# avishkarsaha/learning-adaptive-neighborhoods-for-gnns

Measured on AMD Instinct MI355X. Metric: DGG adj-build+SpMM fwd/bwd edges/sec & achieved HBM GB/s, N=100k d=128 k=32, higher is better.
Workload: dtype f32; 1 GPU; synthetic all-pairs DGG N=100000 d=128 h=64 k~32.3 K=64, u-v-dist/x/k_times_edge_prob, Gumbel(0,0.3) perturbation, + normalize + GCNConv(128,64), fwd+bwd; nodes=100000, feat=128, latent=64, parallelism=row-shard x1, rows_per_rank=100000, hipgraph=True, noise=ranked

## Files before the change

### learning-adaptive-neighborhoods-for-gnns_amd/csrc/dgg_scatter.hip

```cpp
#include "dgg_common.h"
#include "dgg_api_internal.h"
#include "../../include/dgg_hip_next.h"

using namespace dgg;

namespace {

constexpr int BS = 128;
constexpr int PR = 256;

struct PartHdr {
    int *bstart, *cursor;
    int2 *tmp;
    int *slot;
    int2 *recs;
    int *cstart;
};
__host__ __device__ inline size_t align256(size_t x) { return (x + 255) / 256 * 256; }
inline PartHdr part_layout(void *ws, int64_t nb, int64_t nrec) {
    char *w = reinterpret_cast<char *>(ws);
    PartHdr p;
    p.bstart = reinterpret_cast<int *>(w);
    p.cursor = reinterpret_cast<int *>(w + align256((size_t)(nb + 1) * 4));
    p.tmp = reinterpret_cast<int2 *>(w + align256((size_t)(nb + 1) * 4) + align256((size_t)nb * 4));
// ... 70 lines not shown

__global__ __launch_bounds__(1024) void part_sort(const int *__restrict__ bstart, const int2 *__restrict__ tmp, int K,
                                                 int2 *__restrict__ recs, int *__restrict__ slotmap) {
    __shared__ int cnt[BS], base[BS];
    const int tid = threadIdx.x, b = blockIdx.x;
    const int e0 = bstart[b], e1 = bstart[b + 1];
    if (tid < BS) cnt[tid] = 0;
    __syncthreads();
    for (int e = e0 + tid; e < e1; e += 1024) atomicAdd(&cnt[tmp[e].y - b * BS], 1);
    __syncthreads();
    if (tid < 64) {
        const int c0 = cnt[2 * tid], c1 = cnt[2 * tid + 1];
        int incl = c0 + c1;
#pragma unroll
        for (int off = 1; off < 64; off <<= 1) {
            const int v = __shfl_up(incl, off, 64);
            if (tid >= off) incl += v;
        }
        base[2 * tid] = incl - c0 - c1;
        base[2 * tid + 1] = incl - c1;
    }
    __syncthreads();
    if (tid < BS) cnt[tid] = 0;
    __syncthreads();
    for (int e = e0 + tid; e < e1; e += 1024) {
        const int2 rec = tmp[e];
        const int jl = rec.y - b * BS;
        const int pos = e0 + base[jl] + atomicAdd(&cnt[jl], 1);
        recs[pos] = rec;
        slotmap[(int64_t)(rec.x >> 6) * K + (rec.x & 63)] = pos;
    }
}

__global__ void part_chunk_starts(const int *__restrict__ bstart, int nb, const int2 *__restrict__ recs, int nchunks, int chunk,
                                  int *__restrict__ cstart) {
    const int c = blockIdx.x * blockDim.x + threadIdx.x;
    if (c > nchunks) return;
    const int nnz = bstart[nb];
    const int64_t x = (int64_t)c * chunk;
    int e = x < nnz ? (int)x : nnz;
    if (e > 0) {
        const int lim = e + 48 < nnz ? e + 48 : nnz;
        while (e < lim && recs[e].y == recs[e - 1].y) e++;
        if (e < nnz && recs[e].y == recs[e - 1].y) e = (int)x;
    }
    cstart[c] = e;
}

__global__ __launch_bounds__(1024) void part_scan(int *__restrict__ bstart, int *__restrict__ cursor, int nb) {
    __shared__ int part[1024];
    const int tid = threadIdx.x;
    const int per = (nb + 1023) / 1024;
    const int lo = tid * per, hi = lo + per < nb ? lo + per : nb;
    int s = 0;
    for (int b = lo; b < hi; b++) s += cursor[b];
    part[tid] = s;
    __syncthreads();
    for (int off = 1; off < 1024; off <<= 1) {
        int v = tid >= off ? part[tid - off] : 0;
        __syncthreads();
        part[tid] += v;
        __syncthreads();
    }
    int run = part[tid] - s;
    for (int b = lo; b < hi; b++) {
        const int c = cursor[b];
        bstart[b] = run;
        cursor[b] = run;
        run += c;
    }
    if (tid == 1023) bstart[nb] = part[1023];
}

struct SoftkArgs {
    const float *k, *rs, *dA, *da;
    int mode, normalized;
    float *dval_out, *dk;
    const float *ahat_rows;
    float4 *rowinfo;
    const int *recpos;
    const float *dA_rec;
    const float *ainv;
};
template <int H, int R0, int NB>
__device__ __forceinline__ float edge_rows_group(const float *__restrict__ xp, int64_t gi, int K, int lane, int32_t jl, bool myact,
                                                 bool mine, float gl, float vl, float t, int perturb, const float4 xi, float4 &acc) {
    constexpr int LPR = H / 4, NPI = 64 / LPR, r0 = R0;
    const int c4 = lane % LPR, slot = lane / LPR;
    float4 xj[NB];
#pragma unroll
    for (int b = 0; b < NB; b++) {
        const int r = r0 + b * NPI + slot;
        const int rr = r < 64 ? r : 63;
        const int32_t jb = __shfl(jl, rr, 64);
        const bool ab = __shfl((int)myact, rr, 64) != 0 && r < K;
        xj[b] = *reinterpret_cast<const float4 *>(xp + (ab ? (int64_t)jb : gi) * H + 4 * c4);
    }
    float myd2 = 0.0f;
#pragma unroll
    for (int b = 0; b < NB; b++) {
        const float4 d = make_float4(xi.x - xj[b].x, xi.y - xj[b].y, xi.z - xj[b].z, xi.w - xj[b].w);
        float d2 = d.x * d.x + d.y * d.y + d.z * d.z + d.w * d.w;
        if (LPR > 16) d2 += __uint_as_float(xor_shfl<16>(__float_as_uint(d2), lane));
        if (LPR > 8) d2 += __uint_as_float(xor_shfl<8>(__float_as_uint(d2), lane));
        if (LPR > 4) d2 += __uint_as_float(xor_shfl<4>(__float_as_uint(d2), lane));
        if (LPR > 2) d2 += __uint_as_float(xor_shfl<2>(__float_as_uint(d2), lane));
        d2 += __uint_as_float(xor_shfl<1>(__float_as_uint(d2), lane));
        const float tq = __shfl(d2, (lane % NPI) * LPR, 64);
        if ((lane - r0) / NPI == b && mine) myd2 = tq;
    }
    float mydd = 0.0f;
    if (mine && myact && myd2 != 0.0f) {
        const float dist = sqrtf(myd2);
        const float p = c_exp(t * dist);
        const float dp = perturb ? gl * vl / (p + 1e-8f) : gl;
        mydd = dp * t * p / dist;
    }
#pragma unroll
    for (int b = 0; b < NB; b++) {
        const int r = r0 + b * NPI + slot;
        const float dd = __shfl(mydd, r < 64 ? r : 63, 64);
        const float4 d = make_float4(xi.x - xj[b].x, xi.y - xj[b].y, xi.z - xj[b].z, xi.w - xj[b].w);
        acc.x += dd * d.x; acc.y += dd * d.y; acc.z += dd * d.z; acc.w += dd * d.w;
    }
    return mydd;
}
template <int H, int R0, int NBT, int NB = NBT>
__device__ __forceinline__ float edge_rows_pick(int nbat, const float *__restrict__ xp, int64_t gi, int K, int lane, int32_t jl,
                                                bool myact, bool mine, float gl, float vl, float t, int perturb, const float4 xi, float4 &acc) {
    constexpr int STEP = NBT > 8 ? NBT / 8 : 1;
    if constexpr (NB > STEP) {
        if (nbat <= NB - STEP) return edge_rows_pick<H, R0, NBT, NB - STEP>(nbat, xp, gi, K, lane, jl, myact, mine, gl, vl, t, perturb, xi, acc);
    }
    return edge_rows_group<H, R0, NB>(xp, gi, K, lane, jl, myact, mine, gl, vl, t, perturb, xi, acc);
}

template <int H, bool COEF, int R0>
__device__ __forceinline__ void edge_rows_half(const float *__restrict__ xp, int64_t gi, int K, int lane, int32_t jl, bool myact, float gl, float vl,
                                               float t, int perturb, const float4 xi, float4 &acc, float &mycoef) {
    constexpr int NPI = 64 / (H / 4), NBT = 32 / NPI;
    const bool mine = lane >= R0 && lane < R0 + 32;
    const unsigned long long actmask = __ballot(mine && myact);
    if (actmask == 0ull) return;
    const int nbat = (63 - __clzll(actmask) - R0) / NPI + 1;
    const float mydd = edge_rows_pick<H, R0, NBT>(nbat, xp, gi, K, lane, jl, myact, mine, gl, vl, t, perturb, xi, acc);
    if (COEF && mine) mycoef = mydd;
}

template <int H, bool FUSE, bool PAY = false>
__global__ __launch_bounds__(256) void edge_bwd_rows(const float *__restrict__ xp, int64_t rows, const int32_t *__restrict__ idx,
                                                     const float *__restrict__ val, const float *__restrict__ dval, int K,
                                                     int64_t row0, float t, int perturb, const int *__restrict__ slotmap,
                                                     float *__restrict__ coef, float *__restrict__ dxp, SoftkArgs sk) {
    constexpr int LPR = H / 4;
    constexpr int NPI = 64 / LPR;
    const int lane = threadIdx.x & 63, c4 = lane % LPR, slot = lane / LPR;
    const int64_t i = (int64_t)blockIdx.x * 4 + dgg::wave_id();
    if (i >= rows) return;
    const int64_t gi = row0 + i;
    const int32_t jl = lane < K ? idx[i * K + lane] : -1;
    const float vl = lane < K ? val[i * K + lane] : 0.0f;
    float gl;
    if (FUSE) {
        const int lc = lane < K ? lane : K - 1;
        const bool viamap = PAY && sk.recpos != nullptr;
        float dw = viamap ? 0.0f : sk.dA[i * K + lc];
        const int rpos = viamap ? sk.recpos[i * 64 + lc] : 0;
        const bool live = lane < K && jl >= 0;
        if (sk.normalized) {
            const float rsi = sk.rs[gi];
            const int64_t jx = jl >= 0 ? jl : gi;
            const float ai = __fdiv_rn(1.0f, c_sqrt(rsi));
            const float aj = (PAY && sk.ainv) ? sk.ainv[jx] : __fdiv_rn(1.0f, c_sqrt(sk.rs[jx]));
            float dai = sk.da[gi];
            if (sk.ahat_rows) {
                const float ah = lane < K ? sk.ahat_rows[i * K + lane] : 0.0f;
                if (viamap) dw = sk.dA_rec[ah != 0.0f ? rpos : 0];
                if (PAY && ah == 0.0f) dw = 0.0f;
                float rp = dw * ah;
                rp = wave_sum_dpp(rp, lane);
                dai += rp * sqrtf(rsi);
            }
            const float drs = -0.5f * dai * ai / rsi;
            dw = dw * ai * aj + drs;
            if (PAY && lane == 0) sk.rowinfo[i] = make_float4(ai, drs, sk.k[i], 0.0f);
        } else if (PAY && lane == 0) {
            sk.rowinfo[i] = make_float4(1.0f, 0.0f, sk.k[i], 0.0f);
        }
        const float th = c_tanh((float)lane - sk.k[i]);
        const float f = 1.0f - 0.5f * (1.0f + th);
        const float dfdk = 0.5f * (1.0f - th * th);
        gl = (live && sk.mode == 0) ? dw * f : 0.0f;
        float skp = live ? (sk.mode == 0 ? dw * vl * dfdk : dw * dfdk) : 0.0f;
#pragma unroll
        for (int off = 32; off >= 1; off >>= 1) skp += __shfl_xor(skp, off, 64);
        if (lane == 0) sk.dk[i] = skp;
        if (sk.dval_out && lane < K) sk.dval_out[i * K + lane] = gl;
    } else {
        gl = lane < K ? dval[i * K + lane] : 0.0f;
    }
    const float4 xi = *reinterpret_cast<const float4 *>(xp + gi * H + 4 * c4);
    float4 acc = make_float4(0.0f, 0.0f, 0.0f, 0.0f);
    float mycoef = 0.0f;
    constexpr int NBT = (32 / NPI) < 1 ? 1 : 32 / NPI;
    const bool myact = lane < K && jl >= 0 && gl != 0.0f;
    static_assert(NBT * NPI == 32, "two groups of 32 entries");
    edge_rows_half<H, !PAY, 0>(xp, gi, K, lane, jl, myact, gl, vl, t, perturb, xi, acc, mycoef);
    if (K > 32) edge_rows_half<H, !PAY, 32>(xp, gi, K, lane, jl, myact, gl, vl, t, perturb, xi, acc, mycoef);
#pragma unroll
    for (int off = LPR; off < 64; off <<= 1) {
        acc.x += __shfl_xor(acc.x, off, 64); acc.y += __shfl_xor(acc.y, off, 64);
        acc.z += __shfl_xor(acc.z, off, 64); acc.w += __shfl_xor(acc.w, off, 64);
    }
    if (slot == 0) *reinterpret_cast<float4 *>(dxp + gi * H + 4 * c4) = acc;
    if (!PAY && lane < K) {
        const int sl = slotmap[i * K + lane];
        if (sl >= 0) coef[sl] = mycoef;
    }
}

template <int H>
__global__ __launch_bounds__(256) void edge_bwd_rows_chunked(const float *__restrict__ xp, int64_t rows, const int32_t *__restrict__ cptr,
                                                             const int32_t *__restrict__ idx, const float *__restrict__ val, int64_t row0,
                                                             float t, int perturb, float *__restrict__ dxp, SoftkArgs sk) {
    constexpr int LPR = H / 4;
    constexpr int NPI = 64 / LPR;
    constexpr int NBT = (32 / NPI) < 1 ? 1 : 32 / NPI;
    const int lane = threadIdx.x & 63, c4 = lane % LPR, slot = lane / LPR;
    const int64_t i = (int64_t)blockIdx.x * 4 + dgg::wave_id();
    if (i >= rows) return;
    const int64_t gi = row0 + i;
    const int cb = __builtin_amdgcn_readfirstlane(cptr[i]), ce = __builtin_amdgcn_readfirstlane(cptr[i + 1]);
    const float ki = sk.k[i];
    float ai = 1.0f, drs = 0.0f;
    if (sk.normalized) {
        const float rsi = sk.rs[gi];
        ai = __fdiv_rn(1.0f, c_sqrt(rsi));
        float dai = sk.da[gi];
        if (sk.ahat_rows) {
            float rp = 0.0f;
            for (int c = cb; c < ce; c++) {
                const float ah = sk.ahat_rows[(int64_t)c * 64 + lane];
                float dw = sk.dA[(int64_t)c * 64 + lane];
                if (ah == 0.0f) dw = 0.0f;
                rp += dw * ah;
            }
            rp = wave_sum_dpp(rp, lane);
            dai += rp * sqrtf(rsi);
        }
        drs = -0.5f * dai * ai / rsi;
    }
    const float4 xi = *reinterpret_cast<const float4 *>(xp + gi * H + 4 * c4);
    float4 acc = make_float4(0.0f, 0.0f, 0.0f, 0.0f);
    float skp = 0.0f;
    for (int c = cb; c < ce; c++) {
        const int64_t e = (int64_t)c * 64 + lane;
        const int32_t jl = idx[e];
        const float vl = val[e];
        const bool live = jl >= 0;
        float dw = sk.dA[e];
        const float kshift = ki - (float)(64 * (c - cb));
        if (sk.normalized) {
            const int64_t jx = live ? jl : gi;
            const float aj = sk.ainv ? sk.ainv[jx] : __fdiv_rn(1.0f, c_sqrt(sk.rs[jx]));
            if (sk.ahat_rows && sk.ahat_rows[e] == 0.0f) dw = 0.0f;
            dw = dw * ai * aj + drs;
        }
        if (lane == 0) sk.rowinfo[c] = make_float4(ai, drs, kshift, 0.0f);
        const float th = c_tanh((float)lane - kshift);
        const float f = 1.0f - 0.5f * (1.0f + th);
        const float dfdk = 0.5f * (1.0f - th * th);
        const float gl = (live && sk.mode == 0) ? dw * f : 0.0f;
        skp += live ? (sk.mode == 0 ? dw * vl * dfdk : dw * dfdk) : 0.0f;
        const bool myact = live && gl != 0.0f;
        if (__ballot(myact) == 0ull) continue;
        for (int r0 = 0; r0 < 64; r0 += NBT * NPI) {
            const bool mine = lane >= r0 && lane < r0 + NBT * NPI;
            if (__ballot(mine && myact) == 0ull) continue;
            float4 xj[NBT];
#pragma unroll
            for (int b = 0; b < NBT; b++) {
                const int r = r0 + b * NPI + slot;
                const int rr = r < 64 ? r : 63;
                const int32_t jb = __shfl(jl, rr, 64);
                const bool ab = __shfl((int)myact, rr, 64) != 0 && r < 64;
                xj[b] = *reinterpret_cast<const float4 *>(xp + (ab ? (int64_t)jb : gi) * H + 4 * c4);
            }
            float myd2 = 0.0f;
#pragma unroll
            for (int b = 0; b < NBT; b++) {
                const float4 d = make_float4(xi.x - xj[b].x, xi.y - xj[b].y, xi.z - xj[b].z, xi.w - xj[b].w);
// ... 395 lines not shown

template <int H, int R0, int NB>
__device__ __forceinline__ void edge_walk_group(const float *__restrict__ xp, int64_t j, const int4 myrec, const float mydval,
                                                const float4 xj, int64_t row0, float t, int perturb, int lane, int wide, float4 &acc) {
    constexpr int LPR = H / 4, NPI = 64 / LPR, NBT = (32 / NPI) < 1 ? 1 : 32 / NPI;
    const int c4 = lane % LPR, slot = lane / LPR;
    constexpr int r0 = R0;
    const bool mine = lane >= r0 && lane < r0 + NBT * NPI;
    float4 xi[NB];
#pragma unroll
    for (int b = 0; b < NB; b++) {
        const int q = r0 + b * NPI + slot;
        const int src = __shfl(myrec.x, q, 64);
        const int dst = __shfl(myrec.y, q, 64);
        xi[b] = *reinterpret_cast<const float4 *>(xp + (dst >= 0 ? row0 + (wide ? dst : (src >> 6)) : j) * H + 4 * c4);
    }
    float myd2 = 0.0f;
#pragma unroll
    for (int b = 0; b < NB; b++) {
        const float4 d = make_float4(xi[b].x - xj.x, xi[b].y - xj.y, xi[b].z - xj.z, xi[b].w - xj.w);
        float d2 = d.x * d.x + d.y * d.y + d.z * d.z + d.w * d.w;
        if (LPR > 16) d2 += __uint_as_float(xor_shfl<16>(__float_as_uint(d2), lane));
        if (LPR > 8) d2 += __uint_as_float(xor_shfl<8>(__float_as_uint(d2), lane));
        if (LPR > 4) d2 += __uint_as_float(xor_shfl<4>(__float_as_uint(d2), lane));
        d2 += __uint_as_float(xor_shfl<2>(__float_as_uint(d2), lane));
        d2 += __uint_as_float(xor_shfl<1>(__float_as_uint(d2), lane));
        const float tq = __shfl(d2, (lane % NPI) * LPR, 64);
        if ((lane - r0) / NPI == b && mine) myd2 = tq;
    }
    float mydd = 0.0f;
    if (mine && mydval != 0.0f && myd2 != 0.0f) {
        const float dist = sqrtf(myd2);
        const float p = c_exp(t * dist);
        const float dp = perturb ? mydval * __int_as_float(myrec.w) / (p + 1e-8f) : mydval;
        mydd = dp * t * p / dist;
    }
#pragma unroll
    for (int b = 0; b < NB; b++) {
        const float dd = __shfl(mydd, r0 + b * NPI + slot, 64);
        const float4 d = make_float4(xi[b].x - xj.x, xi[b].y - xj.y, xi[b].z - xj.z, xi[b].w - xj.w);
        acc.x -= dd * d.x; acc.y -= dd * d.y; acc.z -= dd * d.z; acc.w -= dd * d.w;
    }
}
template <int H, int R0, int NBT, int NB = NBT>
__device__ __forceinline__ void edge_walk_pick(int nbat, const float *__restrict__ xp, int64_t j, const int4 myrec, const float mydval,
                                               const float4 xj, int64_t row0, float t, int perturb, int lane, int wide, float4 &acc) {
    constexpr int STEP = NBT > 8 ? NBT / 8 : 1;
    if constexpr (NB > STEP) {
        if (nbat <= NB - STEP) return edge_walk_pick<H, R0, NBT, NB - STEP>(nbat, xp, j, myrec, mydval, xj, row0, t, perturb, lane, wide, acc);
    }
    edge_walk_group<H, R0, NB>(xp, j, myrec, mydval, xj, row0, t, perturb, lane, wide, acc);
}

template <int H>
__device__ __forceinline__ void edge_bwd_walk(const float *__restrict__ xp, int64_t j, int pb, int pe, int p1, const int4 *__restrict__ recs,
                                              const float *__restrict__ dA_rec, const float4 *__restrict__ rowinfo, const float4 xj, const float aj,
                                              int64_t row0, float t, int perturb, int lane, float4 &acc, const int wide = 0) {
    constexpr int LPR = H / 4, NPI = 64 / LPR, NBT = (32 / NPI) < 1 ? 1 : 32 / NPI, PER = NBT * NPI;
    static_assert(2 * PER == WALK_BLOCK, "two groups per block");
    for (int e0 = pb; e0 < pe; e0 += WALK_BLOCK) {
        const int nrec = pe - e0 < WALK_BLOCK ? pe - e0 : WALK_BLOCK;
        const bool have = lane < nrec;
        const int ec = have ? e0 + lane : p1 - 1;
        int4 myrec = recs[ec];
        if (!have) myrec.y = -1;
        float mydval;
        {
            const float4 info = rowinfo[myrec.x >> 6];
            const float dw = dA_rec[ec] * info.x * aj + info.y;
            const float th = c_tanh((float)(myrec.x & 63) - info.z);
            mydval = have ? dw * (1.0f - 0.5f * (1.0f + th)) : 0.0f;
        }
        const int n0 = nrec < PER ? nrec : PER;
        edge_walk_pick<H, 0, NBT>((n0 + NPI - 1) / NPI, xp, j, myrec, mydval, xj, row0, t, perturb, lane, wide, acc);
        if (nrec > PER) edge_walk_pick<H, PER, NBT>((nrec - PER + NPI - 1) / NPI, xp, j, myrec, mydval, xj, row0, t, perturb, lane, wide, acc);
    }
#pragma unroll
    for (int off = LPR; off < 64; off <<= 1) {
        acc.x += __shfl_xor(acc.x, off, 64); acc.y += __shfl_xor(acc.y, off, 64);
        acc.z += __shfl_xor(acc.z, off, 64); acc.w += __shfl_xor(acc.w, off, 64);
    }
}

template <int H>
__global__ __launch_bounds__(256) void edge_bwd_node(const float *__restrict__ xp, int64_t ncols, const int *__restrict__ nodeptr,
                                                     const int4 *__restrict__ recs, const float *__restrict__ dA_rec,
                                                     const float4 *__restrict__ rowinfo, const float *__restrict__ rs, int normalized,
                                                     int64_t row0, int64_t rows, float t, int perturb, float *__restrict__ dxp, int out_act,
                                                     unsigned nmain = 0, int wide = 0) {
    constexpr int LPR = H / 4, PER = WALK_BLOCK;
    __shared__ float4 part[4][LPR];
    const int lane = threadIdx.x & 63, c4 = lane % LPR, slot = lane / LPR, wave = dgg::wave_id();
    const bool longmode = nmain != 0 && blockIdx.x >= nmain;
    const int64_t j = longmode ? (int64_t)(blockIdx.x - nmain) : (int64_t)blockIdx.x * 4 + wave;
    if (j >= ncols) return;
    const int p0 = nodeptr[j], p1 = nodeptr[j + 1];
    const bool islong = nmain != 0 && p1 - p0 > NODE_LONG;
    if (islong != longmode) return;
    const float4 xj = *reinterpret_cast<const float4 *>(xp + j * H + 4 * c4);
    const float aj = normalized ? __fdiv_rn(1.0f, c_sqrt(rs[j])) : 1.0f;
    float4 acc = make_float4(0.0f, 0.0f, 0.0f, 0.0f);
    if (!longmode) {
        edge_bwd_walk<H>(xp, j, p0, p1, p1, recs, dA_rec, rowinfo, xj, aj, row0, t, perturb, lane, acc, wide);
    } else {
        const int chunk = ((p1 - p0 + 4 * PER - 1) / (4 * PER)) * PER;
        const int pb = p0 + wave * chunk, pe = pb + chunk < p1 ? pb + chunk : p1;
        edge_bwd_walk<H>(xp, j, pb < p1 ? pb : p1, pe, p1, recs, dA_rec, rowinfo, xj, aj, row0, t, perturb, lane, acc, wide);
        if (slot == 0) part[wave][c4] = acc;
        __syncthreads();
        if (wave != 0) return;
        acc = part[0][c4];
#pragma unroll
        for (int w_ = 1; w_ < 4; w_++) {
            const float4 v = part[w_][c4];
            acc.x += v.x; acc.y += v.y; acc.z += v.z; acc.w += v.w;
        }
    }
    if (slot == 0) {
        float4 *o = reinterpret_cast<float4 *>(dxp + j * H + 4 * c4);
        if (j >= row0 && j < row0 + rows) {
            float4 v = *o;
            acc.x += v.x; acc.y += v.y; acc.z += v.z; acc.w += v.w;
        }
        if (out_act == 1) {
            acc.x *= xj.x > 0.0f ? 1.0f : 0.01f; acc.y *= xj.y > 0.0f ? 1.0f : 0.01f;
            acc.z *= xj.z > 0.0f ? 1.0f : 0.01f; acc.w *= xj.w > 0.0f ? 1.0f : 0.01f;
        }
        *o = acc;
    }
}

template <int F, int NBT>
__global__ __launch_bounds__(256) void conv_bwd_nodeg(const float *__restrict__ G, const float *__restrict__ Hm, int K, int64_t ncols,
                                                      const int *__restrict__ nodeptr, const int4 *__restrict__ recs,
                                                      const float *__restrict__ rs, float *__restrict__ dA, float *__restrict__ dA_rec,
                                                      float *__restrict__ dH, float *__restrict__ da) {
    constexpr int LPR = F / 4, NPW = 64 / LPR;
    const int lane = threadIdx.x & 63, c4 = lane % LPR;
    const int64_t jraw = ((int64_t)blockIdx.x * 4 + dgg::wave_id()) * NPW + lane / LPR;
    const bool live = jraw < ncols;
    const int64_t j = live ? jraw : ncols - 1;
    const int p0 = nodeptr[j], p1 = live ? nodeptr[j + 1] : p0;
    const float4 hj = *reinterpret_cast<const float4 *>(Hm + j * F + 4 * c4);
    const float rsj = rs[j];
    const float aj = __fdiv_rn(1.0f, c_sqrt(rsj));
    float4 acc = make_float4(0.0f, 0.0f, 0.0f, 0.0f);
    float sda = 0.0f;
    int trips = (p1 - p0 + NBT - 1) / NBT;
#pragma unroll
    for (int off = LPR; off < 64; off <<= 1) trips = max(trips, __shfl_xor(trips, off, 64));
    for (int it = 0, e0 = p0; it < trips; it++, e0 += NBT) {
        int src[NBT];
        float cf[NBT];
        float4 g[NBT];
#pragma unroll
        for (int b = 0; b < NBT; b++) {
            const bool have = e0 + b < p1;
            const int4 r = recs[have ? e0 + b : (p1 > p0 ? p1 - 1 : 0)];
            src[b] = have ? r.x : -1;
            cf[b] = have ? __fmul_rn(__int_as_float(r.z), aj) : 0.0f;
            g[b] = *reinterpret_cast<const float4 *>(G + (int64_t)(have ? (r.x >> 6) : 0) * F + 4 * c4);
        }
#pragma unroll
        for (int b = 0; b < NBT; b++) {
            float dot = g[b].x * hj.x;
            dot = fmaf(g[b].y, hj.y, dot); dot = fmaf(g[b].z, hj.z, dot); dot = fmaf(g[b].w, hj.w, dot);
            if (LPR > 16) dot += __uint_as_float(xor_shfl<16>(__float_as_uint(dot), lane));
            if (LPR > 8) dot += __uint_as_float(xor_shfl<8>(__float_as_uint(dot), lane));
            if (LPR > 4) dot += __uint_as_float(xor_shfl<4>(__float_as_uint(dot), lane));
            dot += __uint_as_float(xor_shfl<2>(__float_as_uint(dot), lane));
            dot += __uint_as_float(xor_shfl<1>(__float_as_uint(dot), lane));
            if (src[b] >= 0 && c4 == (b % LPR)) {
                if (dA) __hip_atomic_store(&dA[(int64_t)(src[b] >> 6) * K + (src[b] & 63)], dot, __ATOMIC_RELAXED, __HIP_MEMORY_SCOPE_AGENT);
                dA_rec[e0 + b] = dot;
            }
            acc.x = fmaf(cf[b], g[b].x, acc.x); acc.y = fmaf(cf[b], g[b].y, acc.y);
            acc.z = fmaf(cf[b], g[b].z, acc.z); acc.w = fmaf(cf[b], g[b].w, acc.w);
            sda = fmaf(dot, cf[b], sda);
        }
    }
    if (!live) return;
    *reinterpret_cast<float4 *>(dH + j * F + 4 * c4) = acc;
    if (da && c4 == 0) da[j] = sda * sqrtf(rsj);
}

template <int H, int NBT>
__global__ __launch_bounds__(256) void edge_bwd_nodeg(const float *__restrict__ xp, int64_t ncols, const int *__restrict__ nodeptr,
                                                      const int4 *__restrict__ recs, const float *__restrict__ dA_rec,
                                                      const float4 *__restrict__ rowinfo, const float *__restrict__ rs, int normalized,
                                                      int64_t row0, int64_t rows, float t, int perturb, float *__restrict__ dxp, int out_act) {
// ... 659 lines not shown
    if (dgg_partp_ws_bytes(rows, K, ncols) == 0 || !ws) return refuse(DGG_ERR_UNSUPPORTED, entry, "unsupported size or NULL workspace");
    const bool count_only = stages == PP_COUNT;
    uintptr_t aligned = reinterpret_cast<uintptr_t>(idx) | reinterpret_cast<uintptr_t>(w);
    if (count_only) {
        if (!rs_all || !idx || !w) return refuse(DGG_ERR_ARG, entry, "phase 3 (count) needs idx, w and rs_all");
        if (chunked) aligned |= reinterpret_cast<uintptr_t>(ahat);
    } else {
        if (!val || !rs_rows || (chunked && !cnode))
            return refuse(DGG_ERR_ARG, entry, chunked ? "the payload needs the scores, the row sums and the chunk nodes" : "the payload needs the scores and the row sums");
        if ((stages & PP_RECORDS_ONLY) && (!rs_all || ahat)) return refuse(DGG_ERR_ARG, entry, "phases 4 and 5 (records only) take rs_all and no ahat");
        if (!(stages & PP_RECORDS_ONLY) && (rs_all == nullptr) != (ahat == nullptr)) return refuse(DGG_ERR_ARG, entry, "rs_all and ahat go together");
        aligned |= reinterpret_cast<uintptr_t>(val) | reinterpret_cast<uintptr_t>(ahat);
    }
    if (K == 64 && aligned % 16) return refuse(DGG_ERR_ARG, entry, "idx / w / val / ahat must be 16-byte aligned");
    if (rows == 0) return 0;
    PartP2 p;
    partp2_layout(p, ws, rows, K, ncols);
    hipStream_t st = (hipStream_t)stream;
    switch (pp_threads()) {
        case 256: pp_launch<256>(stages, p, idx, w, val, rs_rows, rows, K, ncols, rs_all, ahat, cnode, st); break;
        case 512: pp_launch<512>(stages, p, idx, w, val, rs_rows, rows, K, ncols, rs_all, ahat, cnode, st); break;
        default: pp_launch<1024>(stages, p, idx, w, val, rs_rows, rows, K, ncols, rs_all, ahat, cnode, st); break;
    }
    return dgg_check_launch(entry);
}

int dgg_partp_build(const int32_t *idx, const float *w, const float *val, const float *rs_rows, int64_t rows, int K, int64_t ncols,
                    void *ws, void *stream) {
    return partp_build_impl("partp_build", idx, w, val, rs_rows, rows, K, ncols, nullptr, nullptr, nullptr, false, ws, 0, stream);
}

int dgg_partp_build_norm(const int32_t *idx, const float *w, const float *val, const float *rs_rows, int64_t rows, int K, int64_t ncols,
                         const float *rs_all, float *ahat, void *ws, void *stream) {
    return partp_build_impl("partp_build_norm", idx, w, val, rs_rows, rows, K, ncols, rs_all, ahat, nullptr, false, ws, 0, stream);
}

int dgg_partp_build_phase(const int32_t *idx, const float *w, const float *val, const float *rs_rows, int64_t rows, int K, int64_t ncols,
                          const float *rs_all, float *ahat, void *ws, int phase, void *stream) {
    return partp_build_impl("partp_build_phase", idx, w, val, rs_rows, rows, K, ncols, rs_all, ahat, nullptr, false, ws, phase, stream);
}
int dgg_partp_build_chunked(const int32_t *idx, const float *w, const float *val, const float *rs_nodes, int64_t chunks, const int32_t *cnode,
                            int64_t ncols, const float *rs_all, float *ahat, void *ws, int phase, void *stream) {
    return partp_build_impl("partp_build_chunked", idx, w, val, rs_nodes, chunks, 64, ncols, rs_all, ahat, cnode, true, ws, phase, stream);
}

int dgg_partp_has_map(int64_t rows) { return pp_builds_map(rows) ? 1 : 0; }

}
int dgg_partp_internal_ptrs(const void *partp_ws, int64_t rows, int K, int64_t ncols, const int **nodeptr, const int **recpos) {
    if (!partp_ws || dgg_partp_ws_bytes(rows, K, ncols) == 0 || !pp_builds_map(rows)) return 1;
    PartP2 p;
    partp2_layout(p, const_cast<void *>(partp_ws), rows, K, ncols);
    *nodeptr = p.nodeptr;
    *recpos = p.recpos;
    return 0;
}
const float *dgg_partp_ainv(const void *partp_ws, int64_t rows, int K, int64_t ncols) {
    if (!partp_ws || dgg_partp_ws_bytes(rows, K, ncols) == 0) return nullptr;
    PartP2 p;
    partp2_layout(p, const_cast<void *>(partp_ws), rows, K, ncols);
    return p.ainv;
}
extern "C" {
int dgg_partp_describe(int64_t rows, int K, int64_t ncols, int64_t *out6) {
    if (!out6 || dgg_partp_ws_bytes(rows, K, ncols) == 0) return dgg_set_error(DGG_ERR_UNSUPPORTED, "partp_describe: no payload partition for this shape");
    PartP2 p;
    partp2_layout(p, nullptr, rows, K, ncols);
    out6[0] = reinterpret_cast<char *>(p.bstart) - static_cast<char *>(nullptr);
    out6[1] = reinterpret_cast<char *>(p.nodeptr) - static_cast<char *>(nullptr);
    out6[2] = reinterpret_cast<char *>(p.recs) - static_cast<char *>(nullptr);
    out6[3] = p.nb;
    out6[4] = p.width;
    out6[5] = pp_threads() / 4;
    return 0;
}

static bool node_split(int64_t ncols) {
    static const int forced = [] { const char *e = getenv("DGG_NODE_SPLIT"); return e ? atoi(e) : -1; }();
    return forced >= 0 ? forced != 0 : ncols <= NODE_SPLIT_MAX;
}
static bool node_groups(int64_t nrec, int64_t ncols) {
    static const int forced = [] { const char *e = getenv("DGG_NODE_GROUPS"); return e ? atoi(e) : -1; }();
    return forced >= 0 ? forced != 0 : nrec < 16 * ncols;
}

static int conv_bwd_partp_impl(const char *entry, bool chunked, const float *G, const float *H, int64_t rows, int K, int F, const void *partp_ws,
                               int64_t ncols, const float *rs, const float *dA_ext, float *dA, float *dA_rec, float *dH, float *da,
                               void *stream) {
    if ((F != 16 && F != 32 && F != 64 && F != 128) || (reinterpret_cast<uintptr_t>(G) % 16) || (reinterpret_cast<uintptr_t>(H) % 16) ||
        (reinterpret_cast<uintptr_t>(dH) % 16))
        return refuse(DGG_ERR_UNSUPPORTED, entry, "feature width must be 16, 32, 64 or 128 (16-byte aligned rows)");
    if (!rs || !partp_ws || !dA_rec || (chunked && !dA) || dgg_partp_ws_bytes(rows, K, ncols) == 0) return refuse(DGG_ERR_ARG, entry, "missing operand");
    if (rows == 0) return 0;
    PartP2 p;
    partp2_layout(p, const_cast<void *>(partp_ws), rows, K, ncols);
    hipStream_t st = (hipStream_t)stream;
    const bool grouped = !chunked && !dA_ext && node_groups(rows * K, ncols);
    const unsigned nmain = (unsigned)((ncols + 3) / 4);
    const bool split = node_split(ncols);
    const dim3 gridn(split ? nmain + (unsigned)ncols : nmain);
    const int wide = chunked ? 1 : 0;
#define DGG_CONV_COLS_P(FF)                                                                                                \
    if (dA_ext)                                                                                                            \
        hipLaunchKernelGGL((conv_bwd_node<FF, true>), gridn, dim3(256), 0, st, G, H, K, ncols, p.nodeptr, p.recs,          \
                           rs, dA, dA_rec, dH, da, dA_ext, split ? nmain : 0u, wide);                                      \
    else if (grouped)                                                                                                      \
        hipLaunchKernelGGL((conv_bwd_nodeg<FF, 4>), dim3((unsigned)((ncols + 4 * (256 / FF) - 1) / (4 * (256 / FF)))), dim3(256), 0, st, G, H, K, \
                           ncols, p.nodeptr, p.recs, rs, dA, dA_rec, dH, da);                                              \
    else                                                                                                                   \
        hipLaunchKernelGGL((conv_bwd_node<FF, false>), gridn, dim3(256), 0, st, G, H, K, ncols, p.nodeptr, p.recs,         \
                           rs, dA, dA_rec, dH, da, (const float *)nullptr, split ? nmain : 0u, wide)
    switch (F) {
        case 16: DGG_CONV_COLS_P(16); break;
        case 32: DGG_CONV_COLS_P(32); break;
        case 64: DGG_CONV_COLS_P(64); break;
        default: DGG_CONV_COLS_P(128); break;
    }
#undef DGG_CONV_COLS_P
    return dgg_check_launch(entry);
}

int dgg_ell_conv_bwd_partp(const float *G, const float *H, int64_t rows, int K, int F, const void *partp_ws, int64_t ncols,
                           const float *rs, float *dA, float *dA_rec, float *dH, float *da, void *stream) {
    return conv_bwd_partp_impl("ell_conv_bwd_partp", false, G, H, rows, K, F, partp_ws, ncols, rs, nullptr, dA, dA_rec, dH, da, stream);
}
int dgg_ell_conv_bwd_partp_ext(const float *G, const float *H, int64_t rows, int K, int F, const void *partp_ws, int64_t ncols,
                               const float *rs, const float *dA_ext, float *dA, float *dA_rec, float *dH, float *da, void *stream) {
    return conv_bwd_partp_impl("ell_conv_bwd_partp_ext", false, G, H, rows, K, F, partp_ws, ncols, rs, dA_ext, dA, dA_rec, dH, da, stream);
}
int dgg_ell_conv_bwd_partp_chunked(const float *G, const float *H, int64_t chunks, int F, const void *partp_ws, int64_t ncols, const float *rs,
                                   const float *dA_ext, float *dA, float *dA_rec, float *dH, float *da, void *stream) {
    return conv_bwd_partp_impl("ell_conv_bwd_partp_chunked", true, G, H, chunks, 64, F, partp_ws, ncols, rs, dA_ext, dA, dA_rec, dH, da, stream);
}

static int edge_bwd_partp_impl(const char *entry, bool chunked, const float *xp, int64_t rows, const int32_t *cptr, int64_t chunks, int h,
                               const int32_t *idx, const float *val, const float *k, const float *rs, const float *dA, const float *dA_rec,
                               const float *da, const float *ahat_rows, int K, int64_t row0, float t, int perturb, int mode, int normalized,
                               const void *partp_ws, int64_t ncols, float *rowinfo_ws, float *dk, float *dxp, int out_act, int phase,
                               int ainv_table, void *stream) {
    if (phase < 0 || phase > 2) return refuse(DGG_ERR_ARG, entry, "phase is 0 (all), 1 (rows) or 2 (nodes)");
    if (mode != 0 && mode != 1) return refuse(DGG_ERR_ARG, entry, "mode must be 0 (k_times) or 1 (k_only)");
    if (out_act != 0 && (out_act != 1 || mode != 0))
        return refuse(DGG_ERR_ARG, entry, "out_act is 0 or 1 (LeakyReLU), mode 0 only");
    if (!k || !dA_rec || !dk || !rowinfo_ws || (normalized && (!rs || !da)) || (chunked && (!cptr || !dA)))
        return refuse(DGG_ERR_ARG, entry, "missing operand");
    if (!dA && !(normalized && ahat_rows))
        return refuse(DGG_ERR_ARG, entry, "dA may be NULL only in the normalised form with ahat_rows");
    if (!dA && !pp_builds_map(rows))
        return refuse(DGG_ERR_ARG, entry, "dA is NULL but the partition of a block this large carries no slot -> record map (dgg_partp_has_map)");
    if (ahat_rows && !normalized) return refuse(DGG_ERR_ARG, entry, "ahat_rows is an operand of the normalised form");
    if (!partp_ws || dgg_partp_ws_bytes(chunks, K, ncols) == 0) return refuse(DGG_ERR_ARG, entry, "no partition");
    if (rows == 0) return 0;
    hipStream_t st = (hipStream_t)stream;
    PartP2 p;
    partp2_layout(p, const_cast<void *>(partp_ws), chunks, K, ncols);
    const SoftkArgs sk{k, rs, dA, da, mode, normalized, nullptr, dk, ahat_rows, reinterpret_cast<float4 *>(rowinfo_ws),
                       dA ? nullptr : p.recpos, dA_rec, (ainv_table && normalized) ? p.ainv : nullptr};
    const unsigned gr = (unsigned)((rows + 3) / 4);
    const bool grouped = !chunked && node_groups(rows * K, ncols);
    const unsigned nmain = (unsigned)((ncols + 3) / 4);
    const bool split = node_split(ncols);
    const int wide = chunked ? 1 : 0;
#define DGG_EDGE_PARTP(HH)                                                                                                  \
    if (phase != 2 && chunked)                                                                                               \
        hipLaunchKernelGGL((edge_bwd_rows_chunked<HH>), dim3(gr), dim3(256), 0, st, xp, rows, cptr, idx, val, row0, t, perturb, dxp, sk); \
    else if (phase != 2)                                                                                                     \
        hipLaunchKernelGGL((edge_bwd_rows<HH, true, true>), dim3(gr), dim3(256), 0, st, xp, rows, idx, val, nullptr, K, row0, t, perturb, nullptr, \
                           nullptr, dxp, sk);                                                                                \
    if (phase == 1 || mode != 0) {                                                                                           \
    } else if (grouped)                                                                                                      \
        hipLaunchKernelGGL((edge_bwd_nodeg<HH, 4>), dim3((unsigned)((ncols + 4 * (256 / HH) - 1) / (4 * (256 / HH)))), dim3(256), 0, st, xp, \
                           ncols, p.nodeptr, p.recs, dA_rec, reinterpret_cast<const float4 *>(rowinfo_ws), rs, normalized, row0, rows, t, \
                           perturb, dxp, out_act);                                                                           \
    else                                                                                                                     \
        hipLaunchKernelGGL(edge_bwd_node<HH>, dim3(split ? nmain + (unsigned)ncols : nmain), dim3(256), 0, st, xp, ncols, p.nodeptr, p.recs, \
                           dA_rec, reinterpret_cast<const float4 *>(rowinfo_ws), rs, normalized, row0, rows, t, perturb, dxp, out_act,  \
                           split ? nmain : 0u, wide)
    switch (h) {
        case 16: DGG_EDGE_PARTP(16); break;
        case 32: DGG_EDGE_PARTP(32); break;
        case 64: DGG_EDGE_PARTP(64); break;
        case 128: DGG_EDGE_PARTP(128); break;
        default: return refuse(DGG_ERR_UNSUPPORTED, entry, "latent_dim must be 16, 32, 64 or 128");
    }
#undef DGG_EDGE_PARTP
    return dgg_check_launch(entry);
}

int dgg_softk_edge_bwd_partp(const float *xp, int64_t rows, int h, const int32_t *idx, const float *val, const float *k, const float *rs,
                             const float *dA, const float *dA_rec, const float *da, const float *ahat_rows, int K, int64_t row0, float t,
                             int perturb, int mode, int normalized, const void *partp_ws, int64_t ncols, float *rowinfo_ws, float *dk,
                             float *dxp, int out_act, void *stream) {
    return edge_bwd_partp_impl("softk_edge_bwd_partp", false, xp, rows, nullptr, rows, h, idx, val, k, rs, dA, dA_rec, da, ahat_rows, K, row0, t,
                               perturb, mode, normalized, partp_ws, ncols, rowinfo_ws, dk, dxp, out_act, 0, 0, stream);
}
int dgg_softk_edge_bwd_partp_phase(const float *xp, int64_t rows, int h, const int32_t *idx, const float *val, const float *k, const float *rs,
                                   const float *dA, const float *dA_rec, const float *da, const float *ahat_rows, int K, int64_t row0, float t,
                                   int perturb, int mode, int normalized, const void *partp_ws, int64_t ncols, float *rowinfo_ws, float *dk,
                                   float *dxp, int out_act, int phase, void *stream) {
    return edge_bwd_partp_impl("softk_edge_bwd_partp_phase", false, xp, rows, nullptr, rows, h, idx, val, k, rs, dA, dA_rec, da, ahat_rows, K, row0, t,
                               perturb, mode, normalized, partp_ws, ncols, rowinfo_ws, dk, dxp, out_act, phase, 0, stream);
}
int dgg_softk_edge_bwd_partp_tab(const float *xp, int64_t rows, int h, const int32_t *idx, const float *val, const float *k, const float *rs,
                                 const float *dA, const float *dA_rec, const float *da, const float *ahat_rows, int K, int64_t row0, float t,
                                 int perturb, int mode, int normalized, const void *partp_ws, int64_t ncols, float *rowinfo_ws, float *dk,
                                 float *dxp, int out_act, int phase, int ainv_table, void *stream) {
    return edge_bwd_partp_impl("softk_edge_bwd_partp_tab", false, xp, rows, nullptr, rows, h, idx, val, k, rs, dA, dA_rec, da, ahat_rows, K, row0, t,
                               perturb, mode, normalized, partp_ws, ncols, rowinfo_ws, dk, dxp, out_act, phase, ainv_table, stream);
}
int dgg_softk_edge_bwd_partp_chunked(const float *xp, int64_t rows, const int32_t *cptr, int64_t chunks, int h, const int32_t *idx, const float *val,
                                     const float *k, const float *rs, const float *dA, const float *dA_rec, const float *da, const float *ahat_rows,
                                     int64_t row0, float t, int perturb, int mode, int normalized, const void *partp_ws, int64_t ncols,
                                     float *rowinfo_ws, float *dk, float *dxp, int out_act, int phase, void *stream) {
    return edge_bwd_partp_impl("softk_edge_bwd_partp_chunked", true, xp, rows, cptr, chunks, h, idx, val, k, rs, dA, dA_rec, da, ahat_rows, 64, row0, t,
                               perturb, mode, normalized, partp_ws, ncols, rowinfo_ws, dk, dxp, out_act, phase, 0, stream);
}
int dgg_softk_edge_bwd_partp_chunked_tab(const float *xp, int64_t rows, const int32_t *cptr, int64_t chunks, int h, const int32_t *idx,
                                         const float *val, const float *k, const float *rs, const float *dA, const float *dA_rec,
                                         const float *da, const float *ahat_rows, int64_t row0, float t, int perturb, int mode,
                                         int normalized, const void *partp_ws, int64_t ncols, float *rowinfo_ws, float *dk, float *dxp,
                                         int out_act, int phase, int ainv_table, void *stream) {
    return edge_bwd_partp_impl("softk_edge_bwd_partp_chunked_tab", true, xp, rows, cptr, chunks, h, idx, val, k, rs, dA, dA_rec, da, ahat_rows, 64, row0,
                               t, perturb, mode, normalized, partp_ws, ncols, rowinfo_ws, dk, dxp, out_act, phase, ainv_table, stream);
}

int dgg_partp_gather_rec(const float *dA, int64_t rows, int64_t ncols, const void *partp_ws, float *dA_rec, void *stream) {
    if (!dA || !dA_rec || !partp_ws || dgg_partp_ws_bytes(rows, 64, ncols) == 0) return dgg_set_error(DGG_ERR_ARG, "partp_gather_rec: missing operand or no partition");
    if (rows == 0) return 0;
    PartP2 p;
    partp2_layout(p, const_cast<void *>(partp_ws), rows, 64, ncols);
    hipLaunchKernelGGL(pp_gather_rec, dim3((unsigned)((rows * 64 + 255) / 256)), dim3(256), 0, (hipStream_t)stream, p.bstart, (int)p.nb, p.recs, dA, dA_rec);
    return dgg_check_launch("partp_gather_rec");
}

int dgg_norm_bwd_da_part(const int32_t *idx, const float *w, const float *rs, const float *dA, int64_t rows, int K, int64_t row0,
                         const void *part_ws, int64_t ncols, float *coef_ws, float *da, void *stream) {
    hipStream_t st = (hipStream_t)stream;
    if (rows == 0) return 0;
    const int64_t nb = nbuckets(ncols);
    PartHdr p = part_layout(const_cast<void *>(part_ws), nb, rows * K);
    hipLaunchKernelGGL(norm_da_rows, dim3((unsigned)((rows + 3) / 4)), dim3(256), 0, st, idx, w, rs, dA, rows, K, row0, p.slot, coef_ws, da);
    hipLaunchKernelGGL(norm_da_cols, dim3((unsigned)nb), dim3(256), 0, st, ncols, p.bstart, p.recs, coef_ws, da);
    return dgg_check_launch("norm_bwd_da_part");
}

}
```

Baseline: 2.823 billion edges/s.

## Add row-share gather path for H=64 edge backward row and node kernels

Adds an EdgeRowShare path for latent dim 64 in the edge backward row kernel and the node-walk kernel. Each lane now owns one neighbor entry mapped across the 16-lane row groups, gathers rows with 32-bit byte offsets, and computes distances with intra-row xor shuffles. The chain-rule scalar is then broadcast back for accumulation. The goal is cheaper addressing and less wasted shuffle and gather work per edge. The path is enabled by default for h=64 non-chunked runs and can be turned off with an env var, which adds code complexity and relies on the offsets fitting in 32 bits.

```diff
diff --git a/learning-adaptive-neighborhoods-for-gnns_amd/csrc/dgg_scatter.hip b/learning-adaptive-neighborhoods-for-gnns_amd/csrc/dgg_scatter.hip
--- a/learning-adaptive-neighborhoods-for-gnns_amd/csrc/dgg_scatter.hip
+++ b/learning-adaptive-neighborhoods-for-gnns_amd/csrc/dgg_scatter.hip
@@ -176,6 +176,61 @@
     const float *dA_rec;
     const float *ainv;
 };
+struct EdgeRowShare {
+    static constexpr int H = 64, LPR = 16, NPI = 4, NBT = 8, PER = 32;
+    static __device__ __forceinline__ int rs_entry(int lane) { return (lane % LPR) * NPI + lane / LPR; }
+    template <int B0, int NB, bool REC, int b = 0>
+    static __device__ __forceinline__ void gather(const char *__restrict__ xpc, uint32_t node0, uint32_t selfoff, uint32_t c4off, int f_node,
+                                                  int f_live, float4 (&g)[NB]) {
+        if constexpr (b < NB) {
+            const int node = dgg::row16_lane<B0 + b>(f_node);
+            const int live = dgg::row16_lane<B0 + b>(f_live);
+            const uint32_t off = live >= 0 ? ((node0 + (uint32_t)(REC ? node >> 6 : node)) << 8 | c4off) : selfoff;
+            g[b] = *reinterpret_cast<const float4 *>(xpc + off);
+            gather<B0, NB, REC, b + 1>(xpc, node0, selfoff, c4off, f_node, f_live, g);
+        }
+    }
+    template <int B0, int NB, int SIGN, int b = 0>
+    static __device__ __forceinline__ void dist2(const float4 (&g)[NB], const float4 a, int c4, int lane, float &myd2) {
+        if constexpr (b < NB) {
+            const float4 d = SIGN > 0 ? make_float4(a.x - g[b].x, a.y - g[b].y, a.z - g[b].z, a.w - g[b].w)
+                                      : make_float4(g[b].x - a.x, g[b].y - a.y, g[b].z - a.z, g[b].w - a.w);
+            float d2 = d.x * d.x + d.y * d.y + d.z * d.z + d.w * d.w;
+            d2 += __uint_as_float(xor_shfl<8>(__float_as_uint(d2), lane));
+            d2 += __uint_as_float(xor_shfl<4>(__float_as_uint(d2), lane));
+            d2 += __uint_as_float(xor_shfl<2>(__float_as_uint(d2), lane));
+            d2 += __uint_as_float(xor_shfl<1>(__float_as_uint(d2), lane));
+            if (c4 == B0 + b) myd2 = d2;
+            __builtin_amdgcn_sched_barrier(0);
+            dist2<B0, NB, SIGN, b + 1>(g, a, c4, lane, myd2);
+        }
+    }
+    template <int B0, int NB, int SIGN, int b = 0>
+    static __device__ __forceinline__ void accumulate(const float4 (&g)[NB], const float4 a, float mydd, float4 &acc) {
+        if constexpr (b < NB) {
+            const float dd = __int_as_float(dgg::row16_lane<B0 + b>(__float_as_int(mydd)));
+            if constexpr (SIGN > 0) {
+                const float4 d = make_float4(a.x - g[b].x, a.y - g[b].y, a.z - g[b].z, a.w - g[b].w);
+                acc.x += dd * d.x; acc.y += dd * d.y; acc.z += dd * d.z; acc.w += dd * d.w;
+            } else {
+                const float4 d = make_float4(g[b].x - a.x, g[b].y - a.y, g[b].z - a.z, g[b].w - a.w);
+                acc.x -= dd * d.x; acc.y -= dd * d.y; acc.z -= dd * d.z; acc.w -= dd * d.w;
+            }
+            accumulate<B0, NB, SIGN, b + 1>(g, a, mydd, acc);
+        }
+    }
+    static __device__ __forceinline__ float chain(bool on, float myd2, float g, float v, float t, int perturb) {
+        float mydd = 0.0f;
+        if (on && myd2 != 0.0f) {
+            const float dist = sqrtf(myd2);
+            const float p = c_exp(t * dist);
+            const float dp = perturb ? g * v / (p + 1e-8f) : g;
+            mydd = dp * t * p / dist;
+        }
+        return mydd;
+    }
+};
+
 template <int H, int R0, int NB>
 __device__ __forceinline__ float edge_rows_group(const float *__restrict__ xp, int64_t gi, int K, int lane, int32_t jl, bool myact,
                                                  bool mine, float gl, float vl, float t, int perturb, const float4 xi, float4 &acc) {
@@ -241,7 +296,22 @@
     if (COEF && mine) mycoef = mydd;
 }
 
-template <int H, bool FUSE, bool PAY = false>
+template <int B0, int NB = EdgeRowShare::NBT>
+__device__ __forceinline__ void edge_rows_group_rs(int nbat, const char *__restrict__ xpc, uint32_t selfoff, uint32_t c4off, int c4, int lane, int qj,
+                                                   float qg, float qv, float t, int perturb, const float4 xi, float4 &acc) {
+    using RS = EdgeRowShare;
+    if constexpr (NB > 1) {
+        if (nbat <= NB - 1) return edge_rows_group_rs<B0, NB - 1>(nbat, xpc, selfoff, c4off, c4, lane, qj, qg, qv, t, perturb, xi, acc);
+    }
+    float4 xj[NB];
+    RS::gather<B0, NB, false>(xpc, 0u, selfoff, c4off, qj, qj, xj);
+    float myd2 = 0.0f;
+    RS::dist2<B0, NB, 1>(xj, xi, c4, lane, myd2);
+    const float mydd = RS::chain(c4 >= B0 && c4 < B0 + RS::NBT && qj >= 0, myd2, qg, qv, t, perturb);
+    RS::accumulate<B0, NB, 1>(xj, xi, mydd, acc);
+}
+
+template <int H, bool FUSE, bool PAY = false, bool RS = false>
 __global__ __launch_bounds__(256) void edge_bwd_rows(const float *__restrict__ xp, int64_t rows, const int32_t *__restrict__ idx,
                                                      const float *__restrict__ val, const float *__restrict__ dval, int K,
                                                      int64_t row0, float t, int perturb, const int *__restrict__ slotmap,
@@ -299,8 +369,21 @@
     constexpr int NBT = (32 / NPI) < 1 ? 1 : 32 / NPI;
     const bool myact = lane < K && jl >= 0 && gl != 0.0f;
     static_assert(NBT * NPI == 32, "two groups of 32 entries");
-    edge_rows_half<H, !PAY, 0>(xp, gi, K, lane, jl, myact, gl, vl, t, perturb, xi, acc, mycoef);
-    if (K > 32) edge_rows_half<H, !PAY, 32>(xp, gi, K, lane, jl, myact, gl, vl, t, perturb, xi, acc, mycoef);
+    if constexpr (RS) {
+        static_assert(H == EdgeRowShare::H && FUSE && PAY, "the row-share body is the payload partition's, H = 64");
+        const int e = EdgeRowShare::rs_entry(lane);
+        const int qj = __shfl(myact ? jl : -1, e, 64);
+        const float qg = __shfl(gl, e, 64), qv = __shfl(vl, e, 64);
+        const unsigned long long actmask = __ballot(myact);
+        const char *xpc = reinterpret_cast<const char *>(xp);
+        const uint32_t c4off = 16u * (uint32_t)c4, selfoff = (uint32_t)gi << 8 | c4off;
+        const unsigned lo = (unsigned)actmask, hi = (unsigned)(actmask >> 32);
+        if (lo) edge_rows_group_rs<0>((31 - __clz(lo)) / NPI + 1, xpc, selfoff, c4off, c4, lane, qj, qg, qv, t, perturb, xi, acc);
+        if (hi) edge_rows_group_rs<8>((31 - __clz(hi)) / NPI + 1, xpc, selfoff, c4off, c4, lane, qj, qg, qv, t, perturb, xi, acc);
+    } else {
+        edge_rows_half<H, !PAY, 0>(xp, gi, K, lane, jl, myact, gl, vl, t, perturb, xi, acc, mycoef);
+        if (K > 32) edge_rows_half<H, !PAY, 32>(xp, gi, K, lane, jl, myact, gl, vl, t, perturb, xi, acc, mycoef);
+    }
 #pragma unroll
     for (int off = LPR; off < 64; off <<= 1) {
         acc.x += __shfl_xor(acc.x, off, 64); acc.y += __shfl_xor(acc.y, off, 64);
@@ -862,7 +945,78 @@
     }
 }
 
-template <int H>
+template <int NB = EdgeRowShare::NBT>
+__device__ __forceinline__ void edge_walk_second_rs(int nbat, const char *__restrict__ xpc, uint32_t row0, uint32_t selfoff, uint32_t c4off, int c4,
+                                                    int lane, const int4 myrec, float mydval, const float4 xj, float t, int perturb, float4 &acc) {
+    using RS = EdgeRowShare;
+    if constexpr (NB > 1) {
+        if (nbat <= NB - 1) return edge_walk_second_rs<NB - 1>(nbat, xpc, row0, selfoff, c4off, c4, lane, myrec, mydval, xj, t, perturb, acc);
+    }
+    float4 xi[NB];
+    RS::gather<RS::NBT, NB, true>(xpc, row0, selfoff, c4off, myrec.x, myrec.y, xi);
+    float myd2 = 0.0f;
+    RS::dist2<RS::NBT, NB, -1>(xi, xj, c4, lane, myd2);
+    const float mydd = RS::chain(c4 >= RS::NBT && mydval != 0.0f, myd2, mydval, __int_as_float(myrec.w), t, perturb);
+    RS::accumulate<RS::NBT, NB, -1>(xi, xj, mydd, acc);
+}
+template <int NB>
+__device__ __forceinline__ void edge_walk_block_rs(int nrec, int e0, int p1, const char *__restrict__ xpc, uint32_t row0, uint32_t selfoff, uint32_t c4off,
+                                                   int c4, int lane, const int4 *__restrict__ recs, const float *__restrict__ dA_rec,
+                                                   const float4 *__restrict__ rowinfo, const float4 xj, float aj, float t, int perturb, float4 &acc) {
+    using RS = EdgeRowShare;
+    const int myq = RS::rs_entry(lane);
+    const bool have = myq < nrec;
+    const int ec = have ? e0 + myq : p1 - 1;
+    int4 myrec = recs[ec];
+    const float mydA = dA_rec[ec];
+    if (!have) myrec.y = -1;
+    const float4 info = rowinfo[myrec.x >> 6];
+    float4 xi[NB];
+    RS::gather<0, NB, true>(xpc, row0, selfoff, c4off, myrec.x, myrec.y, xi);
+    float mydval;
+    {
+        const float dw = mydA * info.x * aj + info.y;
+        const float th = c_tanh((float)(myrec.x & 63) - info.z);
+        mydval = have ? dw * (1.0f - 0.5f * (1.0f + th)) : 0.0f;
+    }
+    float myd2 = 0.0f;
+    RS::dist2<0, NB, -1>(xi, xj, c4, lane, myd2);
+    const float mydd = RS::chain(c4 < RS::NBT && mydval != 0.0f, myd2, mydval, __int_as_float(myrec.w), t, perturb);
+    RS::accumulate<0, NB, -1>(xi, xj, mydd, acc);
+    if constexpr (NB == RS::NBT) {
+        if (nrec > RS::PER) edge_walk_second_rs((nrec - RS::PER + RS::NPI - 1) / RS::NPI, xpc, row0, selfoff, c4off, c4, lane, myrec, mydval, xj, t, perturb, acc);
+    }
+}
+__device__ __forceinline__ void edge_bwd_walk_rs(const float *__restrict__ xp, int64_t j, int pb, int pe, int p1, const int4 *__restrict__ recs,
+                                                 const float *__restrict__ dA_rec, const float4 *__restrict__ rowinfo, const float4 xj, const float aj,
+                                                 int64_t row0, float t, int perturb, int lane, float4 &acc) {
+    using RS = EdgeRowShare;
+    const int c4 = lane % RS::LPR;
+    const char *xpc = reinterpret_cast<const char *>(xp);
+    const uint32_t c4off = 16u * (uint32_t)c4, selfoff = (uint32_t)j << 8 | c4off, r0 = (uint32_t)row0;
+    for (int e0 = pb; e0 < pe; e0 += WALK_BLOCK) {
+        const int nrec = pe - e0 < WALK_BLOCK ? pe - e0 : WALK_BLOCK;
+#define DGG_RS_BLOCK(NB) edge_walk_block_rs<NB>(nrec, e0, p1, xpc, r0, selfoff, c4off, c4, lane, recs, dA_rec, rowinfo, xj, aj, t, perturb, acc)
+        switch ((nrec + RS::NPI - 1) / RS::NPI) {
+            case 1: DGG_RS_BLOCK(1); break;
+            case 2: DGG_RS_BLOCK(2); break;
+            case 3: DGG_RS_BLOCK(3); break;
+            case 4: DGG_RS_BLOCK(4); break;
+            case 5: DGG_RS_BLOCK(5); break;
+            case 6: DGG_RS_BLOCK(6); break;
+            case 7: DGG_RS_BLOCK(7); break;
+            default: DGG_RS_BLOCK(8); break;
+        }
+#undef DGG_RS_BLOCK
+    }
+#pragma unroll
+    for (int off = RS::LPR; off < 64; off <<= 1) {
+        acc.x += __shfl_xor(acc.x, off, 64); acc.y += __shfl_xor(acc.y, off, 64);
+        acc.z += __shfl_xor(acc.z, off, 64); acc.w += __shfl_xor(acc.w, off, 64);
+    }
+}
+
+template <int H, bool RS = false>
 __global__ __launch_bounds__(256) void edge_bwd_node(const float *__restrict__ xp, int64_t ncols, const int *__restrict__ nodeptr,
                                                      const int4 *__restrict__ recs, const float *__restrict__ dA_rec,
                                                      const float4 *__restrict__ rowinfo, const float *__restrict__ rs, int normalized,
@@ -881,11 +1035,13 @@
     const float aj = normalized ? __fdiv_rn(1.0f, c_sqrt(rs[j])) : 1.0f;
     float4 acc = make_float4(0.0f, 0.0f, 0.0f, 0.0f);
     if (!longmode) {
-        edge_bwd_walk<H>(xp, j, p0, p1, p1, recs, dA_rec, rowinfo, xj, aj, row0, t, perturb, lane, acc, wide);
+        if constexpr (RS) edge_bwd_walk_rs(xp, j, p0, p1, p1, recs, dA_rec, rowinfo, xj, aj, row0, t, perturb, lane, acc);
+        else edge_bwd_walk<H>(xp, j, p0, p1, p1, recs, dA_rec, rowinfo, xj, aj, row0, t, perturb, lane, acc, wide);
     } else {
         const int chunk = ((p1 - p0 + 4 * PER - 1) / (4 * PER)) * PER;
         const int pb = p0 + wave * chunk, pe = pb + chunk < p1 ? pb + chunk : p1;
-        edge_bwd_walk<H>(xp, j, pb < p1 ? pb : p1, pe, p1, recs, dA_rec, rowinfo, xj, aj, row0, t, perturb, lane, acc, wide);
+        if constexpr (RS) edge_bwd_walk_rs(xp, j, pb < p1 ? pb : p1, pe, p1, recs, dA_rec, rowinfo, xj, aj, row0, t, perturb, lane, acc);
+        else edge_bwd_walk<H>(xp, j, pb < p1 ? pb : p1, pe, p1, recs, dA_rec, rowinfo, xj, aj, row0, t, perturb, lane, acc, wide);
         if (slot == 0) part[wave][c4] = acc;
         __syncthreads();
         if (wave != 0) return;
@@ -1711,6 +1867,12 @@
 static bool node_groups(int64_t nrec, int64_t ncols) {
     static const int forced = [] { const char *e = getenv("DGG_NODE_GROUPS"); return e ? atoi(e) : -1; }();
     return forced >= 0 ? forced != 0 : nrec < 16 * ncols;
+}
+
+static bool edge_rowshare(int h, bool chunked, int64_t ncols) {
+    if (h != 64 || chunked || ncols * h * 4 >= (int64_t(1) << 31)) return false;
+    const char *e = getenv("DGG_EDGE_ROWSHARE");
+    return !(e && atoi(e) == 0);
 }
 
 static int conv_bwd_partp_impl(const char *entry, bool chunked, const float *G, const float *H, int64_t rows, int K, int F, const void *partp_ws,
@@ -1790,11 +1952,11 @@
     const unsigned nmain = (unsigned)((ncols + 3) / 4);
     const bool split = node_split(ncols);
     const int wide = chunked ? 1 : 0;
-#define DGG_EDGE_PARTP(HH)                                                                                                  \
+#define DGG_EDGE_PARTP(HH, RSB)                                                                                             \
     if (phase != 2 && chunked)                                                                                               \
         hipLaunchKernelGGL((edge_bwd_rows_chunked<HH>), dim3(gr), dim3(256), 0, st, xp, rows, cptr, idx, val, row0, t, perturb, dxp, sk); \
     else if (phase != 2)                                                                                                     \
-        hipLaunchKernelGGL((edge_bwd_rows<HH, true, true>), dim3(gr), dim3(256), 0, st, xp, rows, idx, val, nullptr, K, row0, t, perturb, nullptr, \
+        hipLaunchKernelGGL((edge_bwd_rows<HH, true, true, RSB>), dim3(gr), dim3(256), 0, st, xp, rows, idx, val, nullptr, K, row0, t, perturb, nullptr, \
                            nullptr, dxp, sk);                                                                                \
     if (phase == 1 || mode != 0) {                                                                                           \
     } else if (grouped)                                                                                                      \
@@ -1802,14 +1964,17 @@
                            ncols, p.nodeptr, p.recs, dA_rec, reinterpret_cast<const float4 *>(rowinfo_ws), rs, normalized, row0, rows, t, \
                            perturb, dxp, out_act);                                                                           \
     else                                                                                                                     \
-        hipLaunchKernelGGL(edge_bwd_node<HH>, dim3(split ? nmain + (unsigned)ncols : nmain), dim3(256), 0, st, xp, ncols, p.nodeptr, p.recs, \
+        hipLaunchKernelGGL((edge_bwd_node<HH, RSB>), dim3(split ? nmain + (unsigned)ncols : nmain), dim3(256), 0, st, xp, ncols, p.nodeptr, p.recs, \
                            dA_rec, reinterpret_cast<const float4 *>(rowinfo_ws), rs, normalized, row0, rows, t, perturb, dxp, out_act,  \
                            split ? nmain : 0u, wide)
     switch (h) {
-        case 16: DGG_EDGE_PARTP(16); break;
-        case 32: DGG_EDGE_PARTP(32); break;
-        case 64: DGG_EDGE_PARTP(64); break;
-        case 128: DGG_EDGE_PARTP(128); break;
+        case 16: DGG_EDGE_PARTP(16, false); break;
+        case 32: DGG_EDGE_PARTP(32, false); break;
+        case 64:
+            if (edge_rowshare(h, chunked, ncols)) { DGG_EDGE_PARTP(64, true); }
+            else { DGG_EDGE_PARTP(64, false); }
+            break;
+        case 128: DGG_EDGE_PARTP(128, false); break;
         default: return refuse(DGG_ERR_UNSUPPORTED, entry, "latent_dim must be 16, 32, 64 or 128");
     }
 #undef DGG_EDGE_PARTP
```

Result: no change. 2.822 billion edges/s (-0.1%).
